# KenanGokdenizAcet/phase-based-motion-manipulation

Hardware: AMD Instinct MI355X
Metric: magnified frames/sec at 1920×1080, 5-level pyramid; achieved HBM GB/s vs peak (higher is better)
Workload: dtype f32

## Files before the change

### phase-based-motion-manipulation_amd/csrc/mm_fft.hpp

```cpp
#pragma once
#include <hip/hip_runtime.h>

namespace mm {

typedef float c2 __attribute__((ext_vector_type(2)));

__host__ __device__ __forceinline__ c2 mk(float x, float y) { c2 r = {x, y}; return r; }
__device__ __forceinline__ c2 add(c2 a, c2 b) { return a + b; }
__device__ __forceinline__ c2 sub(c2 a, c2 b) { return a - b; }
__device__ __forceinline__ c2 scale(c2 a, float s) { return a * s; }

template <int DIR>
__device__ __forceinline__ c2 add_i(c2 x, c2 y)
{
    c2 d;
    if constexpr (DIR > 0)
        asm("v_pk_add_f32 %0, %1, %2 op_sel:[0,1] op_sel_hi:[1,0] neg_lo:[0,1]" : "=v"(d) : "v"(x), "v"(y));
    else
        asm("v_pk_add_f32 %0, %1, %2 op_sel:[0,1] op_sel_hi:[1,0] neg_hi:[0,1]" : "=v"(d) : "v"(x), "v"(y));
    return d;
}
template <int DIR>
__device__ __forceinline__ c2 sub_i(c2 x, c2 y) { return add_i<-DIR>(x, y); }

// ... 45 lines not shown
    x0 = s0 + s1;
    x2 = s0 - s1;
    x1 = add_i<DIR>(d0, t);
    x3 = sub_i<DIR>(d0, t);
}

template <int DIR>
__device__ __forceinline__ void dft8(c2 *v)
{
    constexpr float h = 0.70710678118654752f;
    c2 a0 = v[0] + v[4], b0 = v[0] - v[4];
    c2 a1 = v[1] + v[5], b1 = v[1] - v[5];
    c2 a2 = v[2] + v[6], b2 = v[2] - v[6];
    c2 a3 = v[3] + v[7], b3 = v[3] - v[7];
    b1 = add_i<DIR>(b1, b1) * h;
    b3 = sub_i<DIR>(b3, b3) * (-h);
    dft4<DIR>(a0, a1, a2, a3);
    const c2 s0 = add_i<DIR>(b0, b2), d0 = sub_i<DIR>(b0, b2);
    const c2 s1 = b1 + b3, t = b1 - b3;
    v[0] = a0; v[2] = a1; v[4] = a2; v[6] = a3;
    v[1] = s0 + s1;
    v[5] = s0 - s1;
    v[3] = add_i<DIR>(d0, t);
    v[7] = sub_i<DIR>(d0, t);
}

template <int R, int DIR>
__device__ __forceinline__ void apply_twiddles(c2 *u, c2 w1)
{
    if constexpr (R >= 2) u[1] = mul_tw<DIR>(u[1], w1);
    if constexpr (R >= 4) {
        const c2 w2 = mul(w1, w1);
        const c2 w3 = mul(w2, w1);
        u[2] = mul_tw<DIR>(u[2], w2);
        u[3] = mul_tw<DIR>(u[3], w3);
        if constexpr (R >= 8) {
            const c2 w4 = mul(w2, w2);
            u[4] = mul_tw<DIR>(u[4], w4);
            u[5] = mul_tw<DIR>(u[5], mul(w1, w4));
            u[6] = mul_tw<DIR>(u[6], mul(w2, w4));
            u[7] = mul_tw<DIR>(u[7], mul(w3, w4));
            if constexpr (R >= 16) {
                const c2 w8 = mul(w4, w4);
                u[8] = mul_tw<DIR>(u[8], w8);
                u[9] = mul_tw<DIR>(u[9], mul(w1, w8));
                u[10] = mul_tw<DIR>(u[10], mul(w2, w8));
                u[11] = mul_tw<DIR>(u[11], mul(w3, w8));
                const c2 w12 = mul(w4, w8);
                u[12] = mul_tw<DIR>(u[12], w12);
                u[13] = mul_tw<DIR>(u[13], mul(w1, w12));
                u[14] = mul_tw<DIR>(u[14], mul(w2, w12));
                u[15] = mul_tw<DIR>(u[15], mul(w3, w12));
            }
        }
    }
}

constexpr int fft_passes_v(int log2n) { return log2n / 3 + (log2n % 3 ? 1 : 0); }
constexpr int kTwSlots = 20;
template <int LOG2N> constexpr int fft_passes() { return fft_passes_v(LOG2N); }
constexpr int pass_radix_v(int log2n, int p) { return (p < log2n / 3) ? 8 : (log2n % 3 == 2 ? 4 : 2); }
template <int LOG2N, int P> constexpr int pass_radix() { return pass_radix_v(LOG2N, P); }
constexpr int pass_ns_v(int log2n, int p) { return p == 0 ? 1 : pass_ns_v(log2n, p - 1) * pass_radix_v(log2n, p - 1); }

constexpr int tw_entries_v(int log2n) { return 1 << log2n; }

template <int LOG2N, int P = 1, int TWST = 1>
__device__ __forceinline__ void preload_twiddles(c2 (&wb)[kTwSlots], int t, const c2 *__restrict__ tw)
{
    if constexpr (P < fft_passes<LOG2N>()) {
        constexpr int N = 1 << LOG2N, T = N / 8, R = pass_radix<LOG2N, P>(), B = 8 / R;
        constexpr int NS = pass_ns_v(LOG2N, P), TWS = N / (NS * R);
#pragma unroll
        for (int q = 0; q < B; ++q) wb[P * 4 + q] = tw[((t + q * T) & (NS - 1)) * TWS * TWST];
        preload_twiddles<LOG2N, P + 1, TWST>(wb, t, tw);
    }
}

constexpr int xpad_s(int log2n, int ns) { return log2n < 9 || ns == 1 ? 3 : (ns == 8 ? 5 : 30); }
constexpr int xpad_a(int log2n, int ns) { return log2n < 9 || ns == 1 ? 1 : (ns == 8 ? 4 : 0); }
template <int LOG2N, int NS>
__host__ __device__ constexpr int xpad(int i) { return i + xpad_a(LOG2N, NS) * (i >> xpad_s(LOG2N, NS)); }

template <bool WSYNC>
__device__ __forceinline__ void xsync()
{
    if constexpr (WSYNC) __builtin_amdgcn_wave_barrier();
    else __syncthreads();
}

template <int LOG2N, int P, int DIR, bool WSYNC = false>
__device__ __forceinline__ void fft_pass(c2 (&v)[8], int t, c2 *lds, const c2 (&wb)[kTwSlots])
{
    constexpr int N = 1 << LOG2N, T = N / 8, R = pass_radix<LOG2N, P>(), B = 8 / R;
    constexpr int NS = pass_ns_v(LOG2N, P);
    constexpr bool LAST = P == fft_passes<LOG2N>() - 1;
#pragma unroll
    for (int q = 0; q < B; ++q) {
        const int b = t + q * T;
        c2 u[R];
#pragma unroll
        for (int m = 0; m < R; ++m) u[m] = v[q + m * B];
        if constexpr (NS > 1) apply_twiddles<R, DIR>(u, wb[P * 4 + q]);
        if constexpr (R == 8) dft8<DIR>(u);
        else if constexpr (R == 4) dft4<DIR>(u[0], u[1], u[2], u[3]);
        else dft2<DIR>(u[0], u[1]);
        if constexpr (LAST) {
#pragma unroll
            for (int m = 0; m < R; ++m) v[q + m * B] = u[m];
        } else {
            c2 *row = lds + xpad<LOG2N, NS>((b / NS) * NS * R + (b & (NS - 1)));
#pragma unroll
            for (int m = 0; m < R; ++m) row[xpad<LOG2N, NS>(m * NS)] = u[m];
        }
    }
    if constexpr (!LAST) {
        xsync<WSYNC>();
        if constexpr (T % 32 == 0) {
            const c2 *col = lds + xpad<LOG2N, NS>(t);
#pragma unroll
            for (int j = 0; j < 8; ++j) v[j] = lds_ld(col + xpad<LOG2N, NS>(j * T));
        } else {
#pragma unroll
            for (int j = 0; j < 8; ++j) v[j] = lds_ld(lds + xpad<LOG2N, NS>(t + j * T));
        }
        xsync<WSYNC>();
    }
}

template <int LOG2N, int DIR, int P, bool WSYNC = false>
__device__ __forceinline__ void fft_pass_loop(c2 (&v)[8], int t, c2 *lds, const c2 (&wb)[kTwSlots])
{
    if constexpr (P < fft_passes<LOG2N>()) {
        fft_pass<LOG2N, P, DIR, WSYNC>(v, t, lds, wb);
        fft_pass_loop<LOG2N, DIR, P + 1, WSYNC>(v, t, lds, wb);
    }
}

template <int LOG2N, int DIR>
__device__ __forceinline__ void fft_regs(c2 (&v)[8], int t, c2 *lds, const c2 *__restrict__ tw)
{
    c2 wb[kTwSlots];
    preload_twiddles<LOG2N>(wb, t, tw);
    fft_pass_loop<LOG2N, DIR, 0>(v, t, lds, wb);
}

constexpr bool tw_slot_used(int log2n, int i)
{
    return i / 4 >= 1 && i / 4 < fft_passes_v(log2n) && i % 4 < 8 / pass_radix_v(log2n, i / 4);
}

template <int LOG2N, int DIR>
__device__ __forceinline__ void fft_regs_w(c2 (&v)[8], int t, c2 *lds, const c2 (&wf)[kTwSlots])
{
    fft_pass_loop<LOG2N, DIR, 0>(v, t, lds, wf);
}

constexpr int fft_c_v(int log2n) { return log2n >= 9 && log2n <= 12 ? 1 << (log2n - 9) : 1; }
constexpr int fft_inner_v(int log2n) { return log2n >= 9 ? 9 : log2n; }
constexpr int fft_region_v(int log2n) { return (1 << fft_inner_v(log2n)) + (1 << fft_inner_v(log2n)) / 8; }

constexpr bool tw_slot_used_wl(int log2n, int i)
{
    return fft_c_v(log2n) == 1 ? tw_slot_used(log2n, i)
                               : (i == 4 || i == 8 || (i >= 12 && i < 12 + 8 / fft_c_v(log2n)));
}

template <int LOG2N>
__device__ __forceinline__ int fft_bin(int t, int j)
{
    constexpr int C = fft_c_v(LOG2N), T = (1 << LOG2N) / 8;
    if constexpr (C == 1) return t + j * T;
    else return (t >> 6) + C * ((t & 63) + 64 * j);
}

template <int LOG2N>
__host__ __device__ constexpr int zslot(int f)
{
    constexpr int C = fft_c_v(LOG2N), N = 1 << LOG2N;
    return C == 1 ? f : (f % C) * (N / C + 8) + f / C;
}
template <int LOG2N>
__host__ __device__ constexpr int zslot_h(int e)
{
    constexpr int C = fft_c_v(LOG2N), N = 1 << LOG2N;
    return C == 1 ? e : (e % C) * (N / (2 * C) + 8) + e / C;
}
template <int LOG2N> constexpr int zslot_h_size()
{
    return fft_c_v(LOG2N) == 1 ? (1 << LOG2N) / 2 + 1 : (1 << LOG2N) / 2 + 8 * fft_c_v(LOG2N);
}

template <int LOG2N>
__device__ __forceinline__ void preload_twiddles_wl(c2 (&wb)[kTwSlots], int t, const c2 *__restrict__ tw)
{
    constexpr int C = fft_c_v(LOG2N);
    if constexpr (C == 1) {
        preload_twiddles<LOG2N>(wb, t, tw);
    } else {
        preload_twiddles<9, 1, C>(wb, t & 63, tw);
#pragma unroll
        for (int h = 0; h < 8 / C; ++h) wb[12 + h] = tw[t + 64 * C * h];
    }
}

template <int C, int DIR>
__device__ __forceinline__ void dft_c(c2 *u)
{
    if constexpr (C == 8) dft8<DIR>(u);
    else if constexpr (C == 4) dft4<DIR>(u[0], u[1], u[2], u[3]);
    else dft2<DIR>(u[0], u[1]);
}

// ... 58 lines not shown
```

### phase-based-motion-manipulation_amd/csrc/mm_impl.hpp

```cpp
#pragma once
#if (defined(MM_K2_STAMPS) || defined(MM_K34_STAMPS)) && !defined(MM_ONLY_LOG2N)
#error "stamp builds are one-size builds: compile csrc/mm_api.hip alone with -DMM_ONLY_LOG2N=<log2 N>"
#endif
#include <hip/hip_runtime.h>

#include <algorithm>
#include <cmath>
#include <cstdio>
#include <cstdlib>
#include <cstring>
#include <new>
#include <vector>

#include "../../include/mm.h"
#include "mm_steer.hpp"

using namespace mm;

#define HIPCHK(x)                                                             \
    do {                                                                      \
        hipError_t e_ = (x);                                                  \
        if (e_ != hipSuccess) {                                               \
            if (getenv("MM_DEBUG"))                                           \
                fprintf(stderr, "mm355: %s failed: %s (%s:%d)\n", #x,         \
// ... 451 lines not shown
    }
    for (int i = 1; i < p.levels - 1; ++i) {
        volatile float num = (float)(i - 1), den = (float)(p.levels - 3);
        const float ratio = num / den;
        const float center = p.min_freq * powf(p.max_freq / p.min_freq, 1.0f - ratio);
        const float bwid = center * 0.5f;
        sp.lo[i] = center - bwid;
        sp.hi[i] = center + bwid;
        sp.inv_w[i] = 1.0f / (sp.hi[i] - sp.lo[i]);
    }
}

static bool bands_fit_table(const Spec &sp)
{
    for (int a = 1; a < sp.L - 1; ++a)
        for (int b = a + 1; b < sp.L - 1; ++b)
            for (int c = b + 1; c < sp.L - 1; ++c) {
                const float lo = fmaxf(sp.lo[a], fmaxf(sp.lo[b], sp.lo[c]));
                const float hi = fminf(sp.hi[a], fminf(sp.hi[b], sp.hi[c]));
                if (lo < hi) return false;
            }
    return true;
}

static bool bands_overlap(const Spec &sp)
{
    for (int a = 1; a < sp.L - 1; ++a)
        for (int b = a + 1; b < sp.L - 1; ++b) {
            const float lo = fmaxf(sp.lo[a], sp.lo[b]), hi = fminf(sp.hi[a], sp.hi[b]);
            if (hi - lo > 1e-5f * hi) return true;
        }
    return false;
}

static Blur5 build_blur()
{
    const double c0 = 0.2270270270, c1 = 0.3162162162, c2w = 0.0702702703;
    const double f1 = 0.5 * 1.3846153846, f2 = 0.5 * 3.2307692308 - 1.0;
    Blur5 b;
    b.w0 = (float)(c0 + 2.0 * c1 * (1.0 - f1));
    b.w1 = (float)(c1 * f1 + c2w * (1.0 - f2));
    b.w2 = (float)(c2w * f2);
    return b;
}

static int validate_params(const mm_params *p)
{
    if (!p) return MM_ERR_INVALID;
    if (p->levels < 1 || p->levels > kMaxLevels) return MM_ERR_UNSUPPORTED;
    if (p->mode == MM_MODE_STEERABLE) {
        if (p->orientations != 4 && p->orientations != 6 && p->orientations != 8)
            return MM_ERR_UNSUPPORTED;
        if (p->temporal_filter != MM_FILTER_DIFF && p->temporal_filter != MM_FILTER_IIR)
            return MM_ERR_INVALID;
        if (p->temporal_filter == MM_FILTER_IIR &&
            !(p->iir_low > 0.0f && p->iir_low < p->iir_high && p->iir_high <= 1.0f))
            return MM_ERR_INVALID;
    } else {
        if (p->orientations != 1) return MM_ERR_UNSUPPORTED;
        if (p->mode != MM_MODE_PYRAMID && p->mode != MM_MODE_STANDARD) return MM_ERR_UNSUPPORTED;
    }
    if (p->edge_mode != MM_EDGE_REPEAT && p->edge_mode != MM_EDGE_CLAMP) return MM_ERR_INVALID;
    if (!(p->min_freq > 0.0f) || !(p->max_freq > 0.0f)) return MM_ERR_INVALID;
    return MM_OK;
}

static constexpr int ktab_slots(int log2n)
{
    const int C = fft_c_v(log2n), te = (1 << log2n) / 2 + 1;
    return (te + C - 1) / C * C;
}

static int ilog2(int n)
{
    int l = 0;
    while ((1 << l) < n) ++l;
    return l;
}

template <int LOG2N> static size_t lds_fft_bytes()
{
    return sizeof(c2) * (size_t)groups_per_wg<LOG2N>() * lds_complex<(1 << LOG2N)>();
}
template <int LOG2N>
static int set_attrs(int W)
{
    (void)W;
    if constexpr (LOG2N == 12) {
        const int lds = (int)(sizeof(c2) * 2 * lds_complex<4096>());
        for (int f : {MM_RGBA8, MM_RGBA32F, MM_RGBA16F, MM_RGBA8_SRGB, MM_NV12, MM_P010, MM_Y8, MM_Y16, MM_YUY2})
            MM_FMT_SWITCH(f, HIPCHK(hipFuncSetAttribute(reinterpret_cast<const void *>(&k_rows_inv_compose<12, FMT_>),
                                                        hipFuncAttributeMaxDynamicSharedMemorySize, lds)))
        HIPCHK(hipFuncSetAttribute(reinterpret_cast<const void *>(&k_sb_cols<12>),
                                   hipFuncAttributeMaxDynamicSharedMemorySize, 81920));
    }
    if constexpr (LOG2N == 13) {
        auto set = [](const void *f, size_t b) {
            return b > 65536 ? hipFuncSetAttribute(f, hipFuncAttributeMaxDynamicSharedMemorySize, (int)b)
                             : hipSuccess;
        };
        const size_t x = sizeof(c2) * lds_complex<8192>();
        HIPCHK(set(reinterpret_cast<const void *>(&k_rows_inv<13>), sizeof(c2) * k3_groups<13>() * lds_complex<8192>()));
        HIPCHK(set(reinterpret_cast<const void *>(&k_dbg_cols<13>), 2 * sizeof(c2) * lds_complex<4096>()));
        (void)x;
#define MM_SET_K2(MODE)                                                                                  \
        HIPCHK(set(reinterpret_cast<const void *>(&k_cols<13, MODE>), k2_lds_bytes<13, MODE>()));        \
        HIPCHK(set(reinterpret_cast<const void *>(&k_cols_tail<13, MODE>), k2_lds_bytes<13, MODE>()))
        MM_SET_K2(MM_MODE_PYRAMID);
        MM_SET_K2(MM_MODE_STANDARD);
        MM_SET_K2(MM_K2_PYR_TAB);
#undef MM_SET_K2
    }
    if constexpr (LOG2N == 11) {
        const int lds = (int)(sizeof(c2) * 4 * lds_complex<2048>());
        for (int f : {MM_RGBA8, MM_RGBA32F, MM_RGBA16F, MM_RGBA8_SRGB, MM_NV12, MM_P010, MM_Y8, MM_Y16, MM_YUY2})
            MM_FMT_SWITCH(f, HIPCHK(hipFuncSetAttribute(reinterpret_cast<const void *>(&k_rows_inv_compose4<11, FMT_>),
                                                        hipFuncAttributeMaxDynamicSharedMemorySize, lds)))
    }
    return MM_OK;
}

template <int LOG2N>
static int launch_k1(mm_handle *h, const uint8_t *in, int nframes, const Frames &fr, hipStream_t s, c2 *G)
{
    const int fmt = fr.fmt;
    const int ppf = (h->H + 1) / 2;
    const int total = ppf * nframes;
    const bool lat = (total + k1_groups<LOG2N>() - 1) / k1_groups<LOG2N>() < 512;
    ProfScope ps(h, s, MM_K_ROWS_FWD, nframes);
#define MM_K1_LAUNCH(F, GEN, LAT)                                                                  \
    do {                                                                                           \
        constexpr int gpw = k1_gpw<LOG2N, LAT>();                                                  \
        const size_t lds = sizeof(c2) * (size_t)gpw * lds_complex<(1 << LOG2N)>();                \
        if (lds > 65536)                                                                           \
            HIPCHK(hipFuncSetAttribute(reinterpret_cast<const void *>(&k_rows_fwd<LOG2N, F, GEN, LAT>), \
                                       hipFuncAttributeMaxDynamicSharedMemorySize, (int)lds));     \
        hipLaunchKernelGGL((k_rows_fwd<LOG2N, F, GEN, LAT>), dim3((total + gpw - 1) / gpw),         \
                           dim3(gpw * fft_T<LOG2N>()), lds, s, in, ppf, total, g,                  \
                           h->d_col3, h->d_row3, h->d_col, h->d_row, h->d_tw, G, h->g_stride);     \
    } while (0)
    const bool gen = h->geo.ox || h->geo.oy;
    const Geo g = geo_of(h, fr);
    if (gen) {
        MM_FMT_SWITCH_FULLRES(fmt, MM_K1_LAUNCH(kK1Fmt<FMT_>, true, false))
    } else {
        MM_FMT_SWITCH_K1(fmt, if (lat) MM_K1_LAUNCH(kK1Fmt<FMT_>, false, true);
                              else MM_K1_LAUNCH(kK1Fmt<FMT_>, false, false))
    }
#undef MM_K1_LAUNCH
    HIPCHK(hipGetLastError());
    return MM_OK;
}

template <int LOG2N>
static int launch_k2(mm_handle *h, int nframes, const c2 *Gprev, const c2 *G, hipStream_t s)
{
    const int gpw = k2_groups<LOG2N>();
    const int cols = (1 << LOG2N) / 2;
    const int blocks = (cols + gpw - 1) / gpw;
    static_assert(ktab_slots(LOG2N) == k2_tab_slots<LOG2N>(), "d_ktab column stride");
    const int tab_mode = h->spec.mode == MM_MODE_STANDARD ? MM_MODE_STANDARD : h->k2_tab ? MM_K2_PYR_TAB : -1;
    if (tab_mode >= 0 && h->ktab_mode != tab_mode) {
        const int n = (cols + 1) * k2_tab_slots<LOG2N>();
        if (tab_mode == MM_MODE_STANDARD)
            hipLaunchKernelGGL((k_k2_table<LOG2N, MM_MODE_STANDARD>), dim3((n + 255) / 256), dim3(256), 0, s,
                               h->d_ktab, h->d_kmsum, h->spec);
        else
            hipLaunchKernelGGL((k_k2_table<LOG2N, MM_K2_PYR_TAB>), dim3((n + 255) / 256), dim3(256), 0, s,
                               h->d_ktab, h->d_kmsum, h->spec);
        HIPCHK(hipGetLastError());
        h->ktab_mode = tab_mode;
    }
    ProfScope ps(h, s, MM_K_COLS, nframes);
    int k = nframes >= 24 ? nframes * h->k2_tail_pct / 100 : 0;
    k = std::max(0, std::min(k, nframes - 2));
    const int k2t = nframes >= 24 && blocks >= 2 ? std::min(nframes * h->k2_tail2_pct / 100, nframes - 2) : 0;
    const int tb = k2t > 0 ? blocks / 2 : 0;
#define MM_K2_LAUNCH(MODE)                                                                           \
    do {                                                                                             \
                                         \
        const size_t lds = k2_lds_bytes<LOG2N, MODE>();                                              \
        hipLaunchKernelGGL((k_cols<LOG2N, MODE>), dim3(blocks + tb), dim3(k2_threads<LOG2N>()), lds, s, G, \
                           h->g_stride, Gprev, h->d_Q, h->q_stride, nframes, h->geo, h->spec, h->d_tw, h->d_ktab, \
                           h->d_kmsum, nframes - k, tb, k2t);                                        \
        if (k)                                                                                       \
            hipLaunchKernelGGL((k_cols_tail<LOG2N, MODE>), dim3(k), dim3(k2_threads<LOG2N>()), lds, s, G, \
                               h->g_stride, Gprev, h->d_Q, h->q_stride, nframes - k, h->geo, h->spec, h->d_tw, \
                               h->d_ktab, h->d_kmsum);                                               \
    } while (0)
    if (h->spec.mode == MM_MODE_STANDARD) MM_K2_LAUNCH(MM_MODE_STANDARD);
    else if (h->k2_tab2) MM_K2_LAUNCH(MM_K2_PYR_TAB2);
    else if (h->k2_tab) MM_K2_LAUNCH(MM_K2_PYR_TAB);
    else MM_K2_LAUNCH(MM_MODE_PYRAMID);
#undef MM_K2_LAUNCH
    HIPCHK(hipGetLastError());
    return MM_OK;
}

static int ensure_frames(mm_handle *h, void **buf, int *have, int frames, size_t per_frame, hipStream_t s)
{
    if (*buf && *have >= frames) return MM_OK;
    void *p = nullptr;
    if (h_alloc(h, &p, per_frame * (size_t)frames) != hipSuccess) return MM_ERR_OOM;
    h_retire(h, *buf, s, true);
    *buf = p;
    *have = frames;
    return MM_OK;
}
static int ensure_yh(mm_handle *h, hipStream_t s)
{
    return ensure_frames(h, reinterpret_cast<void **>(&h->d_Yh), &h->yh_frames, h->chunk,
                         sizeof(float) * h->yh_stride, s);
}

static int place_batch(mm_handle *h, int n, hipStream_t s, int *base)
{
    *base = 0;
    if (!h->g_valid) return MM_OK;
    if (h->gs + 1 + n <= h->chunk + 1) {
        *base = h->gs + 1;
        return MM_OK;
    }
    if (n > h->gs) {
        HIPCHK(hipMemcpyAsync(h->d_G + h->g_stride * h->chunk, h->d_G + h->g_stride * h->gs,
                              sizeof(c2) * h->g_stride, hipMemcpyDeviceToDevice, s));
        h->gs = h->chunk;
    }
    return MM_OK;
}

static int launch_k4(mm_handle *h, const uint8_t *in, uint8_t *out, int frame0, int nframes,
                     const Frames &fr, hipStream_t s);

static bool nv12_quads_aligned(const uint8_t *in, const uint8_t *out, const Frames &fr, int nframes)
{
    const uintptr_t a = reinterpret_cast<uintptr_t>(in) + fr.in.c_off, b = reinterpret_cast<uintptr_t>(out);
    uintptr_t m = a | fr.in.c_pitch | b | fr.out.pitch | (b + fr.out.c_off) | fr.out.c_pitch;
    if (nframes > 1) m |= fr.in.stride | fr.out.stride;
    return (m & 3u) == 0;
}
static bool mono_quads_aligned(const uint8_t *out, const Frames &fr, int nframes)
{
    uintptr_t m = reinterpret_cast<uintptr_t>(out) | fr.out.pitch;
    if (nframes > 1) m |= fr.out.stride;
    return (m & 3u) == 0;
}
static bool k34_fits(const mm_handle *h, const uint8_t *in, const uint8_t *out, const Frames &fr, int nframes)
{
    if (fmt_nv12(fr.fmt) && !nv12_quads_aligned(in, out, fr, nframes)) return false;
    if (fmt_mono(fr.fmt) && !mono_quads_aligned(out, fr, nframes)) return false;
    const Geo &g = h->geo;
    return g.N <= 4096 &&
           !g.ox && !g.oy && g.W % 8 == 0 && g.x0 >= 4 && g.x0 % 4 == 0 &&
           g.x0 + g.W + 4 <= g.N && g.N - g.H >= 4 && g.Hn == g.H + 4 && g.rb == g.y0 - 2 &&
           2 * (g.N / 8) >= g.W / 4;
}

#ifndef MM_K34_ROWS_4K
#define MM_K34_ROWS_4K 128
#endif
static int k34_strip_rows(const mm_handle *h, int nout)
{
    if (h->k34_rows >= 0) return h->k34_rows;
    const int cap = h->N >= 4096 ? MM_K34_ROWS_4K : 64;
    const int R = std::min(cap, (int)((long long)h->H * nout / 1024) / 4 * 4);
    return R >= 16 ? R : 0;
}

template <int LOG2N>
static int launch_k3(mm_handle *h, const uint8_t *in, uint8_t *out, int frame0, int nframes,
                     const Frames &fr, hipStream_t s)
{
    const int nout = nframes - frame0;
    if (nout <= 0) return MM_OK;
    const int fmt = fr.fmt;
    const int R = k34_strip_rows(h, nout);
    constexpr int k34o_per_cu = 4 * fft_T<LOG2N>() <= 1024 ? 1024 / (4 * fft_T<LOG2N>()) : 0;
    if constexpr (LOG2N <= 11) if (R == 0 && h->k34_rows < 0 && h->k34_oneshot && k34_fits(h, in, out, fr, nframes) &&
                                   ((LOG2N <= 10 && (h->H + 3) / 4 * nout <= k34o_per_cu * h->num_cu) ||
                                    h->k34_oneshot == 2)) {
        const int strips = (h->H + 3) / 4;
        const size_t lds = sizeof(c2) * 4 * lds_complex<(1 << LOG2N)>();
        const dim3 grid((unsigned)(strips * nout)), block(4 * fft_T<LOG2N>());
        ProfScope ps(h, s, MM_K_ROWS_INV_COMPOSE, nout);
        MM_FMT_SWITCH(fmt, hipLaunchKernelGGL((k_rows_inv_compose4<LOG2N, FMT_>), grid, block, lds, s, h->d_Q,
                                              h->q_stride, in, out, frame0, strips, geo_of(h, fr), h->blur,
                                              h->d_col3, h->d_row3, h->d_tw))
        HIPCHK(hipGetLastError());
        return MM_OK;
    }
    if (R >= 4 && k34_fits(h, in, out, fr, nframes)) {
        const int strips = (h->H + R - 1) / R, steps = R / 4 + 1;
        const size_t lds = sizeof(c2) * 2 * lds_complex<(1 << LOG2N)>();
        const dim3 grid((unsigned)(strips * nout)), block(2 * fft_T<LOG2N>());
        ProfScope ps(h, s, MM_K_ROWS_INV_COMPOSE, nout);
        MM_FMT_SWITCH(fmt, hipLaunchKernelGGL((k_rows_inv_compose<LOG2N, FMT_>), grid, block, lds, s, h->d_Q,
                                              h->q_stride, in, out, frame0, strips, steps, geo_of(h, fr),
                                              h->blur, h->d_col3, h->d_row3, h->d_tw))
        HIPCHK(hipGetLastError());
        return MM_OK;
    }
    const int ppf = h->geo.Hq / 2;
    const int total = ppf * nout;
    const int gpw = k3_groups<LOG2N>();
    int rc = ensure_yh(h, s);
    if (rc) return rc;
    {
        ProfScope ps(h, s, MM_K_ROWS_INV, nout);
        hipLaunchKernelGGL((k_rows_inv<LOG2N>), dim3((total + gpw - 1) / gpw),
                           dim3(k3_threads<LOG2N>()), sizeof(c2) * (size_t)gpw * lds_complex<(1 << LOG2N)>(),
                           s, h->d_Q,
                           h->q_stride, h->d_Yh, h->yh_stride, frame0, ppf, total, h->geo,
                           h->blur, h->d_tw);
        HIPCHK(hipGetLastError());
    }
    return launch_k4(h, in, out, frame0, nframes, fr, s);
}

template <int FMT> static constexpr auto k4_kernel()
{
    if constexpr (kMono<FMT>) return &k_compose_mono<FMT>;
    else return &k_compose<FMT>;
}
static int launch_k4(mm_handle *h, const uint8_t *in, uint8_t *out, int frame0, int nframes,
                     const Frames &fr, hipStream_t s)
{
    const int nout = nframes - frame0;
    if (nout <= 0) return MM_OK;
    const int fmt = fr.fmt;
    if (h->geo.ox || h->geo.oy) {
        const size_t tot = (size_t)nout * h->W * h->H;
        ProfScope ps(h, s, MM_K_COMPOSE, nout);
        const dim3 grid((unsigned)((tot + 255) / 256));
        MM_FMT_SWITCH_FULLRES(fmt, hipLaunchKernelGGL((k_compose_odd<FMT_>), grid, dim3(256), 0, s, h->d_Yh,
                                              h->yh_stride, in, out, frame0, nout, geo_of(h, fr), h->blur,
                                              h->d_col, h->d_row))
        HIPCHK(hipGetLastError());
        return MM_OK;
    }
    const int rt = (h->H + kTileRows - 1) / kTileRows, ct = (h->W + kTileCols - 1) / kTileCols;
    const dim3 grid(rt * ct * nout);
    ProfScope ps(h, s, MM_K_COMPOSE, nout);
    MM_FMT_SWITCH(fmt, hipLaunchKernelGGL((k4_kernel<FMT_>()), grid, dim3(kTileCols), 0, s, h->d_Yh,
                                          h->yh_stride, in, out, frame0, rt, ct, geo_of(h, fr), h->blur,
                                          h->d_col3, h->d_row3))
    HIPCHK(hipGetLastError());
    return MM_OK;
}

static int copy_frames(mm_handle *h, const uint8_t *in, uint8_t *out, int n, const Frames &fr, hipStream_t s)
{
    if (n <= 0) return MM_OK;
    if (fr.packed) {
        HIPCHK(hipMemcpyAsync(out, in, fr.fb * n, hipMemcpyDeviceToDevice, s));
        return MM_OK;
    }
    const unsigned rb = (unsigned)fmt_row_bytes(h->W, fr.fmt);
    const int rows = fmt_420(fr.fmt) ? h->H + h->H / 2 : h->H;
    const Geo g = geo_of(h, fr);
    for (int f0 = 0; f0 < n; f0 += 32768) {
        const dim3 grid((unsigned)rows, (unsigned)std::min(32768, n - f0));
        const uint8_t *src = in + fr.in.stride * f0;
        uint8_t *dst = out + fr.out.stride * f0;
        if (fmt_unit(fr.fmt) == 1) hipLaunchKernelGGL((k_copy_rows<uint8_t>), grid, dim3(256), 0, s, src, dst, g, rb, h->H);
        else if (fmt_unit(fr.fmt) == 2) hipLaunchKernelGGL((k_copy_rows<uint16_t>), grid, dim3(256), 0, s, src, dst, g, rb, h->H);
        else hipLaunchKernelGGL((k_copy_rows<uint32_t>), grid, dim3(256), 0, s, src, dst, g, rb, h->H);
        HIPCHK(hipGetLastError());
    }
    return MM_OK;
}

static int steer_bands(const mm_handle *h)
{
    const int nmid = h->spec.L >= 3 ? h->spec.L - 2 : 0;
    return nmid * (h->spec.O / 2);
}
static int steer_planes(const mm_handle *h) { return h->spec.filt == MM_FILTER_IIR ? 3 : 1; }
static size_t steer_plane_floats(const mm_handle *h)
{
    return (size_t)steer_bands(h) * h->geo.Hn * (h->geo.Wy + 4);
}
// ... 245 lines not shown
```

### phase-based-motion-manipulation_amd/csrc/mm_kernels.hpp

```cpp
#pragma once
#include "mm_fft.hpp"
#include "mm_srgb.hpp"
#include <stdint.h>
#include <type_traits>

namespace mm {

constexpr int kMaxLevels = 16;
constexpr float kPi = 3.14159265359f;

struct Tap4 {
    int idx[4];
    float w[4];
};

struct Geo {
    int W, H, N;
    int x0, y0;
    int ox, oy;
    int Hg;
    int Wy;
    int rb;
    int Hn;
    int Hq;
// ... 1839 lines not shown
                if (r % 2 == 0) {
                    cd0 = cd;
                } else {
                    const c2 v = cd0 + cd;
                    const float mine = X & 1 ? v.y : v.x, send = X & 1 ? v.x : v.y;
                    const float theirs = __builtin_bit_cast(float, __builtin_amdgcn_mov_dpp(
                        __builtin_bit_cast(int, send), 0xB1, 0xF, 0xF, true));
                    if constexpr (kP010<FMT>) {
                        const unsigned cc10 = p010_ccode(mine + theirs, X & 1 ? g.nv.cro : g.nv.cbo);
                        st_off<uint16_t>(outp, g.lo.c_off + (unsigned)(i >> 1) * g.lo.c_pitch + (unsigned)X * 2u,
                                         (uint16_t)(cc10 << 6));
                    } else {
                        const unsigned cc8 = nv12_ccode(mine + theirs, X & 1 ? g.nv.cro : g.nv.cbo);
                        st_off<uint8_t>(outp, g.lo.c_off + (unsigned)(i >> 1) * g.lo.c_pitch + (unsigned)X, (uint8_t)cc8);
                    }
                }
            } else if constexpr (k422<FMT>) {
                static_assert(TC % 2 == 0, "packed 4:2:2: tiles of whole macropixels");
                c2 cd;
                const unsigned yc = nv12_ycode(rr, gg, bb, g, cd);
                const float mine = X & 1 ? cd.y : cd.x, send = X & 1 ? cd.x : cd.y;
                const float theirs = __builtin_bit_cast(float, __builtin_amdgcn_mov_dpp(
                    __builtin_bit_cast(int, send), 0xB1, 0xF, 0xF, true));
                const unsigned cc = nv12_ccode(mine + theirs, X & 1 ? g.nv.cro : g.nv.cbo);
                const unsigned half = yc << (8u * g.lo.yb) | cc << (8u - 8u * g.lo.yb);
                const unsigned other = (unsigned)__builtin_amdgcn_mov_dpp((int)half, 0xB1, 0xF, 0xF, true);
                if (!(X & 1))
                    st_stream<uint32_t>(outp + (size_t)((unsigned)i * g.lo.pitch), (unsigned)X * 2u, half | other << 16);
            } else {
                Pix<FMT>::store(outp + (unsigned)i * g.lo.pitch, (unsigned)X, rr, gg, bb);
            }
        }
    }
}

template <int FMT>
__global__ __launch_bounds__(kTileCols)
void k_compose_mono(const float *__restrict__ Yh, size_t yh_stride, const uint8_t *__restrict__,
                    uint8_t *__restrict__ frames_out, int frame0, int row_tiles,
                    int col_tiles, Geo g, Blur5 bw, const float4 *__restrict__,
                    const float4 *__restrict__)
{
    static_assert(kMono<FMT>, "the 4:2:0 and RGBA formats compose with k_compose");
    constexpr int TR = kTileRows, TC = kTileCols;
    int b = blockIdx.x;
    const int ct = b % col_tiles;
    b /= col_tiles;
    const int rt = b % row_tiles;
    const int frame = frame0 + b / row_tiles;
    const int i0 = rt * TR, X = ct * TC + (int)threadIdx.x;
    if (X >= g.W) return;
    const float *Yf = Yh + (size_t)frame * yh_stride;
    float yv[TR + 4];
#pragma unroll
    for (int v = 0; v < TR + 4; ++v) {
        const int cy = wrap_near(g.y0 + i0 - 2 + v, g.N, g.edge);
        const int k = (cy - g.rb + 2 * g.N) & (g.N - 1);
        const float y = ld_off<float>(Yf, (unsigned)(min(k, g.Hn - 1) * g.Wy + X) * 4u);
        yv[v] = k < g.Hn ? y : 0.0f;
    }
    uint8_t *outp = frames_out + (size_t)frame * g.lo.stride;
#pragma unroll
    for (int r = 0; r < TR; ++r) {
        const int i = i0 + r;
        if (i < g.H) {
            const float yb = bw.w0 * yv[r + 2] + bw.w1 * (yv[r + 1] + yv[r + 3]) +
                             bw.w2 * (yv[r] + yv[r + 4]);
            mono_store<FMT>(outp + (size_t)((unsigned)i * g.lo.pitch), (unsigned)X, sat(yb), g);
        }
    }
}

#ifdef MM_K34_STAMPS
__device__ unsigned long long mm_k34_stamps[65536 * 8];
#define K34_STAMP(i)                                                     \
    do {                                                                 \
        const unsigned long long n_ = __builtin_amdgcn_s_memtime();      \
        st_acc[i] += n_ - st_prev;                                       \
        st_prev = n_;                                                    \
    } while (0)
#else
#define K34_STAMP(i) do { } while (0)
#endif
template <int LOG2N, int FMT>
__global__ __launch_bounds__(2 * fft_T<LOG2N>()) __attribute__((amdgpu_waves_per_eu(4)))
void k_rows_inv_compose(const c2 *__restrict__ Q, size_t q_stride,
                        const uint8_t *__restrict__ frames_in, uint8_t *__restrict__ frames_out,
                        int frame0, int strips, int steps, Geo g, Blur5 bw,
                        const float4 *__restrict__ colW3, const float4 *__restrict__ rowW3,
                        const c2 *__restrict__ tw)
{
    constexpr int N = 1 << LOG2N, T = fft_T<LOG2N>(), TK = q_tile<LOG2N>();
    using raw_t = typename ChromaSrc<FMT>::raw_t;
    constexpr unsigned bpp = LumaSrc<FMT>::bpp;
    extern __shared__ __attribute__((aligned(16))) c2 lds_all[];
    const int grp = T % 64 == 0 ? __builtin_amdgcn_readfirstlane(threadIdx.x / T) : threadIdx.x / T;
    const int t = threadIdx.x % T;
    c2 *lds = lds_all + grp * lds_complex<N>();
    const float *raw_all = reinterpret_cast<const float *>(lds_all);
    constexpr int GROUP_FLOATS = 2 * lds_complex<N>();
    const int b = xcd_remap(blockIdx.x, gridDim.x);
    const int frame = frame0 + b / strips;
    const int i0 = (b % strips) * 4 * (steps - 1);
    const c2 *Qf = Q + (size_t)frame * q_stride;
    const uint8_t *img = frames_in + (size_t)frame * g.li.stride;
    uint8_t *outp = frames_out + (size_t)frame * g.lo.stride;

    const int q = threadIdx.x;
    const bool vq = 4 * q < g.W;
    const int X = vq ? 4 * q : g.W - 4;
    const unsigned cl = (unsigned)wrap_near(X - 1, g.W, g.edge);
    const unsigned cr = (unsigned)wrap_near(X + 4, g.W, g.edge);
    auto chroma_row = [&](int i, c2 (&hc)[4]) {
        if constexpr (!kMono<FMT>) {
            const int row = wrap_near(min(i, g.H), g.H, g.edge);
            c2 a[6];
            if constexpr (k422<FMT>) {
                c422_quad_iq(img, g, row, (unsigned)X, cl, cr, a);
            } else if constexpr (k420<FMT>) {
                const unsigned pl = ld_off<raw_t>(img, c420_off<FMT>(g, row, cl));
                unsigned pm0, pm1;
                c420_quad_pairs<FMT>(img, g, row, (unsigned)X, pm0, pm1);
                const unsigned pr = ld_off<raw_t>(img, c420_off<FMT>(g, row, cr));
                a[0] = c420_iq2<FMT>(pl, g);
                a[1] = a[2] = c420_iq2<FMT>(pm0, g);
                a[3] = a[4] = c420_iq2<FMT>(pm1, g);
                a[5] = c420_iq2<FMT>(pr, g);
            } else {
                const unsigned base = (unsigned)row * (g.li.pitch / bpp);
                raw_t p[6];
                p[0] = ld_off<raw_t>(img, (base + cl) * bpp);
                if constexpr (bpp == 4) {
                    const uint4 m = ld_quad_a4(img, (base + (unsigned)X) * bpp);
                    p[1] = m.x; p[2] = m.y; p[3] = m.z; p[4] = m.w;
                } else {
#pragma unroll
                    for (int k = 0; k < 4; ++k) p[1 + k] = ld_off<raw_t>(img, (base + (unsigned)X + k) * bpp);
                }
                p[5] = ld_off<raw_t>(img, (base + cr) * bpp);
#pragma unroll
                for (int k = 0; k < 6; ++k) a[k] = chroma_iq2<FMT>(p[k]);
            }
#pragma unroll
            for (int k = 0; k < 4; ++k) {
                const float4 wc = colW3[X + k];
                hc[k] = wc.x * a[k] + wc.y * a[k + 1] + wc.z * a[k + 2];
            }
        }
    };

    float yw[8][4];
    [[maybe_unused]] c2 hc[6][4];
    chroma_row(i0 - 1, hc[4]);
    chroma_row(i0, hc[5]);
#ifdef MM_K34_STAMPS
    unsigned long long st_acc[8] = {0, 0, 0, 0, 0, 0, 0, 0};
    unsigned long long st_prev = __builtin_amdgcn_s_memtime();
    st_acc[7] = __builtin_amdgcn_s_memrealtime();
#endif
    float4 qv[8];
    auto load_q = [&](int s_) {
        const int ka_ = i0 + 4 * s_ + 2 * grp;
        const int kl = ka_ < g.Hn ? ka_ : 0;
        const float4 *Qp = reinterpret_cast<const float4 *>(Qf + (size_t)(kl / TK) * g.Qs * TK + (kl % TK));
        const unsigned up = (unsigned)t * (TK / 2), dn = (unsigned)(T - 1 - t) * (TK / 2);
#pragma unroll
        for (int j = 0; j < 8; ++j) {
            if (j < 4) qv[j] = (Qp + (size_t)(j * T) * (TK / 2))[up];
            else qv[j] = (Qp + (size_t)(N - j * T - (T - 1)) * (TK / 2))[dn];
        }
    };
    for (int s = 0; s < steps; ++s) {
        const int ka = i0 + 4 * s + 2 * grp;
        const bool valid = ka < g.Hn;
        load_q(s);
        c2 v[8];
#pragma unroll
        for (int j = 0; j < 8; ++j) {
            const int fq = t + j * T;
            const bool mirror = fq > N / 2;
            const int ff = mirror ? N - fq : fq;
            float4 qq = qv[j];
            if (ff == 0 || ff == N / 2) { qq.y = 0.0f; qq.w = 0.0f; }
            if (mirror) { qq.y = -qq.y; qq.w = -qq.w; }
            v[j] = valid ? mk(qq.x - qq.w, qq.y + qq.z) : mk(0.0f, 0.0f);
        }
        K34_STAMP(0);
        fft_regs<LOG2N, +1>(v, t, lds, tw);
        K34_STAMP(1);
        float *raw = reinterpret_cast<float *>(lds) + kZShift;
#pragma unroll
        for (int j = 0; j < 8; ++j) {
            raw[t + j * T] = fabsf(v[j].x);
            raw[N + t + j * T] = fabsf(v[j].y);
        }
        __syncthreads();
        K34_STAMP(2);
        const float4 *b4 = reinterpret_cast<const float4 *>(raw_all) + ((g.x0 + X) >> 2);
#pragma unroll
        for (int r = 0; r < 4; ++r) {
            const float4 *r4 = b4 + ((r >> 1) * GROUP_FLOATS + (r & 1) * N) / 4;
            const float4 P = r4[0], Z = r4[1];
            yw[4 + r][0] = bw.w0 * P.z + bw.w1 * (P.y + P.w) + bw.w2 * (P.x + Z.x);
            yw[4 + r][1] = bw.w0 * P.w + bw.w1 * (P.z + Z.x) + bw.w2 * (P.y + Z.y);
            yw[4 + r][2] = bw.w0 * Z.x + bw.w1 * (P.w + Z.y) + bw.w2 * (P.z + Z.z);
            yw[4 + r][3] = bw.w0 * Z.y + bw.w1 * (Z.x + Z.z) + bw.w2 * (P.w + Z.w);
        }
        __syncthreads();
        K34_STAMP(3);
        if (s > 0) {
            if constexpr (k420<FMT>) {
#pragma unroll
                for (int k = 0; k < 4; ++k) hc[2][k] = hc[1][k];
                chroma_row(i0 + 4 * s - 2, hc[3]);
#pragma unroll
                for (int k = 0; k < 4; ++k) hc[4][k] = hc[3][k];
                chroma_row(i0 + 4 * s, hc[5]);
            } else {
#pragma unroll
                for (int r = 0; r < 4; ++r) chroma_row(i0 + 4 * s - 3 + r, hc[2 + r]);
            }
            [[maybe_unused]] c2 cd0[4];
            for (int r = 0; r < 4; ++r) {
                K34_STAMP(4);
                const int i = i0 + 4 * s - 4 + r;
                if constexpr (kMono<FMT>) {
                    if (vq && i < g.H) {
                        float yl[4];
#pragma unroll
                        for (int k = 0; k < 4; ++k) {
                            const float yb = bw.w0 * yw[r + 2][k] + bw.w1 * (yw[r + 1][k] + yw[r + 3][k]) +
                                             bw.w2 * (yw[r][k] + yw[r + 4][k]);
                            yl[k] = sat(yb);
                        }
                        mono_store_quad<FMT>(outp + (size_t)((unsigned)i * g.lo.pitch), (unsigned)X, yl, g);
                    }
                } else if (vq && i < g.H) {
                    const float4 wr = rowW3[i];
                    float rr[4], gg[4], bb[4];
#pragma unroll
                    for (int k = 0; k < 4; ++k) {
                        const c2 cc = wr.x * hc[r][k] + wr.y * hc[r + 1][k] + wr.z * hc[r + 2][k];
                        const float yb = bw.w0 * yw[r + 2][k] + bw.w1 * (yw[r + 1][k] + yw[r + 3][k]) +
                                         bw.w2 * (yw[r][k] + yw[r + 4][k]);
                        yiq_rgb(yb, cc, rr[k], gg[k], bb[k]);
                    }
                    [[maybe_unused]] const unsigned o = (unsigned)i * (g.lo.pitch / bpp) + (unsigned)X;
                    if constexpr (k422<FMT>) {
                        c422_store_quad(outp, g, i, X, rr, gg, bb);
                    } else if constexpr (k420<FMT>) {
                        c420_store_quad<FMT>(outp, g, i, X, r & 1, rr, gg, bb, cd0);
                    } else if constexpr (bpp == 4) {
                        uint4 px;
                        px.x = Pix<FMT>::pack(rr[0], gg[0], bb[0]);
                        px.y = Pix<FMT>::pack(rr[1], gg[1], bb[1]);
                        px.z = Pix<FMT>::pack(rr[2], gg[2], bb[2]);
                        px.w = Pix<FMT>::pack(rr[3], gg[3], bb[3]);
                        st_stream_quad_a4(outp + (size_t)((unsigned)i * g.lo.pitch), (unsigned)X * 4u, px);
                    } else {
#pragma unroll
                        for (int k = 0; k < 4; ++k) Pix<FMT>::store(outp, o + k, rr[k], gg[k], bb[k]);
                    }
                }
            }
        }
        K34_STAMP(5);
#pragma unroll
        for (int r = 0; r < 4; ++r)
#pragma unroll
            for (int k = 0; k < 4; ++k) yw[r][k] = yw[4 + r][k];
        if constexpr (!kMono<FMT>) {
#pragma unroll
            for (int k = 0; k < 4; ++k) {
                hc[0][k] = hc[4][k];
                hc[1][k] = hc[5][k];
            }
        }
    }
#ifdef MM_K34_STAMPS
    st_acc[6] = (unsigned long long)steps;
    st_acc[7] = (__builtin_amdgcn_s_memrealtime() - st_acc[7]) << 32 | (st_acc[7] & 0xffffffffull);
    const int w = blockIdx.x * (blockDim.x / 64) + threadIdx.x / 64;
    if (threadIdx.x % 64 == 0 && w < 65536)
        for (int i = 0; i < 8; ++i) mm_k34_stamps[w * 8 + i] = st_acc[i];
#endif
}

template <int LOG2N, int FMT>
__global__ __launch_bounds__(4 * fft_T<LOG2N>())
void k_rows_inv_compose4(const c2 *__restrict__ Q, size_t q_stride,
                         const uint8_t *__restrict__ frames_in, uint8_t *__restrict__ frames_out,
                         int frame0, int strips, Geo g, Blur5 bw,
                         const float4 *__restrict__ colW3, const float4 *__restrict__ rowW3,
                         const c2 *__restrict__ tw)
{
    constexpr int N = 1 << LOG2N, T = fft_T<LOG2N>(), TK = q_tile<LOG2N>();
    using raw_t = typename ChromaSrc<FMT>::raw_t;
    constexpr unsigned bpp = LumaSrc<FMT>::bpp;
    extern __shared__ __attribute__((aligned(16))) c2 lds_all[];
    const int grp = T % 64 == 0 ? __builtin_amdgcn_readfirstlane(threadIdx.x / T) : threadIdx.x / T;
// ... 332 lines not shown
```

Before: 54330.

## Stage RGBA8 source rows into LDS via async global_load_lds during FFT

For RGBA8/sRGB inputs with 16-byte-aligned pitches at N<=4096, the inverse-compose kernel issues global_load_lds DMA for the four upcoming source rows right after the first FFT pass. Chroma reconstruction then reads those rows from LDS, so the global-load latency overlaps with the remaining FFT passes. The FFT syncs become explicit lgkmcnt waits plus s_barrier, so the pending vmcnt DMA is not drained early. In exchange the kernel uses more LDS per workgroup, which may lower occupancy, and it relies on hand-placed waitcnt ordering.

After: 55520 (median of 6 runs). +2.2%, better.

```diff
diff --git a/phase-based-motion-manipulation_amd/csrc/mm_fft.hpp b/phase-based-motion-manipulation_amd/csrc/mm_fft.hpp
--- a/phase-based-motion-manipulation_amd/csrc/mm_fft.hpp
+++ b/phase-based-motion-manipulation_amd/csrc/mm_fft.hpp
@@ -151,14 +151,19 @@
 template <int LOG2N, int NS>
 __host__ __device__ constexpr int xpad(int i) { return i + xpad_a(LOG2N, NS) * (i >> xpad_s(LOG2N, NS)); }
 
-template <bool WSYNC>
+constexpr int kSyncLds = 2;
+template <int WSYNC>
 __device__ __forceinline__ void xsync()
 {
-    if constexpr (WSYNC) __builtin_amdgcn_wave_barrier();
+    if constexpr (WSYNC == kSyncLds) {
+        asm volatile("s_waitcnt lgkmcnt(0)" ::: "memory");
+        __builtin_amdgcn_s_barrier();
+        asm volatile("" ::: "memory");
+    } else if constexpr (WSYNC) __builtin_amdgcn_wave_barrier();
     else __syncthreads();
 }
 
-template <int LOG2N, int P, int DIR, bool WSYNC = false>
+template <int LOG2N, int P, int DIR, int WSYNC = 0>
 __device__ __forceinline__ void fft_pass(c2 (&v)[8], int t, c2 *lds, const c2 (&wb)[kTwSlots])
 {
     constexpr int N = 1 << LOG2N, T = N / 8, R = pass_radix<LOG2N, P>(), B = 8 / R;
@@ -197,7 +202,7 @@
     }
 }
 
-template <int LOG2N, int DIR, int P, bool WSYNC = false>
+template <int LOG2N, int DIR, int P, int WSYNC = 0>
 __device__ __forceinline__ void fft_pass_loop(c2 (&v)[8], int t, c2 *lds, const c2 (&wb)[kTwSlots])
 {
     if constexpr (P < fft_passes<LOG2N>()) {
diff --git a/phase-based-motion-manipulation_amd/csrc/mm_impl.hpp b/phase-based-motion-manipulation_amd/csrc/mm_impl.hpp
--- a/phase-based-motion-manipulation_amd/csrc/mm_impl.hpp
+++ b/phase-based-motion-manipulation_amd/csrc/mm_impl.hpp
@@ -557,12 +557,23 @@
 {
     return sizeof(c2) * (size_t)groups_per_wg<LOG2N>() * lds_complex<(1 << LOG2N)>();
 }
+template <int LOG2N> static size_t k34_lds_bytes(bool srcdma)
+{
+    return sizeof(c2) * 2 * lds_complex<(1 << LOG2N)>() + (srcdma ? (size_t)k34_src_bytes<LOG2N>() : 0);
+}
 template <int LOG2N>
 static int set_attrs(int W)
 {
     (void)W;
+    if constexpr (LOG2N <= 12) if (k34_lds_bytes<LOG2N>(true) > 65536) {
+        const int lds = (int)k34_lds_bytes<LOG2N>(true);
+        HIPCHK(hipFuncSetAttribute(reinterpret_cast<const void *>(&k_rows_inv_compose<LOG2N, MM_RGBA8, true>),
+                                   hipFuncAttributeMaxDynamicSharedMemorySize, lds));
+        HIPCHK(hipFuncSetAttribute(reinterpret_cast<const void *>(&k_rows_inv_compose<LOG2N, MM_RGBA8_SRGB, true>),
+                                   hipFuncAttributeMaxDynamicSharedMemorySize, lds));
+    }
     if constexpr (LOG2N == 12) {
-        const int lds = (int)(sizeof(c2) * 2 * lds_complex<4096>());
+        const int lds = (int)k34_lds_bytes<12>(false);
         for (int f : {MM_RGBA8, MM_RGBA32F, MM_RGBA16F, MM_RGBA8_SRGB, MM_NV12, MM_P010, MM_Y8, MM_Y16, MM_YUY2})
             MM_FMT_SWITCH(f, HIPCHK(hipFuncSetAttribute(reinterpret_cast<const void *>(&k_rows_inv_compose<12, FMT_>),
                                                         hipFuncAttributeMaxDynamicSharedMemorySize, lds)))
@@ -720,6 +731,13 @@
     if (nframes > 1) m |= fr.out.stride;
     return (m & 3u) == 0;
 }
+static bool k34_src_dma(const uint8_t *in, const Frames &fr, int nframes)
+{
+    if (fr.fmt != MM_RGBA8 && fr.fmt != MM_RGBA8_SRGB) return false;
+    uintptr_t m = reinterpret_cast<uintptr_t>(in) | fr.in.pitch;
+    if (nframes > 1) m |= fr.in.stride;
+    return (m & 15u) == 0;
+}
 static bool k34_fits(const mm_handle *h, const uint8_t *in, const uint8_t *out, const Frames &fr, int nframes)
 {
     if (fmt_nv12(fr.fmt) && !nv12_quads_aligned(in, out, fr, nframes)) return false;
@@ -766,12 +784,20 @@
     }
     if (R >= 4 && k34_fits(h, in, out, fr, nframes)) {
         const int strips = (h->H + R - 1) / R, steps = R / 4 + 1;
-        const size_t lds = sizeof(c2) * 2 * lds_complex<(1 << LOG2N)>();
+        const bool dma = LOG2N <= 12 && k34_src_dma(in, fr, nframes);
+        const size_t lds = k34_lds_bytes<LOG2N>(dma);
         const dim3 grid((unsigned)(strips * nout)), block(2 * fft_T<LOG2N>());
         ProfScope ps(h, s, MM_K_ROWS_INV_COMPOSE, nout);
-        MM_FMT_SWITCH(fmt, hipLaunchKernelGGL((k_rows_inv_compose<LOG2N, FMT_>), grid, block, lds, s, h->d_Q,
-                                              h->q_stride, in, out, frame0, strips, steps, geo_of(h, fr),
-                                              h->blur, h->d_col3, h->d_row3, h->d_tw))
+#define MM_K34_LAUNCH(F, DMA)                                                                        \
+        hipLaunchKernelGGL((k_rows_inv_compose<LOG2N, F, DMA>), grid, block, lds, s, h->d_Q,          \
+                           h->q_stride, in, out, frame0, strips, steps, geo_of(h, fr), h->blur,      \
+                           h->d_col3, h->d_row3, h->d_tw)
+        if constexpr (LOG2N <= 12) if (dma) {
+            if (fmt == MM_RGBA8) MM_K34_LAUNCH(MM_RGBA8, true);
+            else MM_K34_LAUNCH(MM_RGBA8_SRGB, true);
+        }
+        if (!dma) MM_FMT_SWITCH(fmt, MM_K34_LAUNCH(FMT_, false))
+#undef MM_K34_LAUNCH
         HIPCHK(hipGetLastError());
         return MM_OK;
     }
diff --git a/phase-based-motion-manipulation_amd/csrc/mm_kernels.hpp b/phase-based-motion-manipulation_amd/csrc/mm_kernels.hpp
--- a/phase-based-motion-manipulation_amd/csrc/mm_kernels.hpp
+++ b/phase-based-motion-manipulation_amd/csrc/mm_kernels.hpp
@@ -1945,7 +1945,9 @@
 #else
 #define K34_STAMP(i) do { } while (0)
 #endif
-template <int LOG2N, int FMT>
+template <int FMT> constexpr bool k34_dma_fmt = FMT == MM_RGBA8 || FMT == MM_RGBA8_SRGB;
+template <int LOG2N> constexpr int k34_src_bytes() { return 4 * 4 * (1 << LOG2N); }
+template <int LOG2N, int FMT, bool SRCDMA = false>
 __global__ __launch_bounds__(2 * fft_T<LOG2N>()) __attribute__((amdgpu_waves_per_eu(4)))
 void k_rows_inv_compose(const c2 *__restrict__ Q, size_t q_stride,
                         const uint8_t *__restrict__ frames_in, uint8_t *__restrict__ frames_out,
@@ -1956,7 +1958,10 @@
     constexpr int N = 1 << LOG2N, T = fft_T<LOG2N>(), TK = q_tile<LOG2N>();
     using raw_t = typename ChromaSrc<FMT>::raw_t;
     constexpr unsigned bpp = LumaSrc<FMT>::bpp;
-    extern __shared__ __attribute__((aligned(16))) c2 lds_all[];
+    static_assert(!SRCDMA || k34_dma_fmt<FMT>, "staged source rows: 4-byte pixels");
+    extern __shared__ __attribute__((aligned(16))) c2 lds_raw[];
+    [[maybe_unused]] const uint8_t *srcl = reinterpret_cast<const uint8_t *>(lds_raw);
+    c2 *lds_all = lds_raw + (SRCDMA ? k34_src_bytes<LOG2N>() / (int)sizeof(c2) : 0);
     const int grp = T % 64 == 0 ? __builtin_amdgcn_readfirstlane(threadIdx.x / T) : threadIdx.x / T;
     const int t = threadIdx.x % T;
     c2 *lds = lds_all + grp * lds_complex<N>();
@@ -2011,6 +2016,35 @@
             }
         }
     };
+    [[maybe_unused]] auto stage_row = [&](int i, int r) {
+        if constexpr (SRCDMA) {
+            typedef __attribute__((address_space(1))) const void gptr_t;
+            typedef __attribute__((address_space(3))) void lptr_t;
+            const int row = i < g.H ? i : (g.edge ? g.H - 1 : 0);
+            const uint8_t *src = img + (size_t)((unsigned)row * g.li.pitch) + (unsigned)X * 4u;
+            const unsigned wbase = (unsigned)__builtin_amdgcn_readfirstlane((int)(threadIdx.x & ~63u)) * 16u;
+            const uint8_t *dst = srcl + r * (4 * N) + wbase;
+            __builtin_amdgcn_global_load_lds((gptr_t *)src, (lptr_t *)dst, 16, 0, 0);
+        }
+    };
+    [[maybe_unused]] auto chroma_row_staged = [&](int r, c2 (&hc)[4]) {
+        if constexpr (SRCDMA) {
+            const uint8_t *rowp = srcl + r * (4 * N);
+            unsigned p[6];
+            p[0] = *reinterpret_cast<const unsigned *>(rowp + cl * 4u);
+            const uint4 m = *reinterpret_cast<const uint4 *>(rowp + (unsigned)X * 4u);
+            p[1] = m.x; p[2] = m.y; p[3] = m.z; p[4] = m.w;
+            p[5] = *reinterpret_cast<const unsigned *>(rowp + cr * 4u);
+            c2 a[6];
+#pragma unroll
+            for (int k = 0; k < 6; ++k) a[k] = chroma_iq2<FMT>(p[k]);
+#pragma unroll
+            for (int k = 0; k < 4; ++k) {
+                const float4 wc = colW3[X + k];
+                hc[k] = wc.x * a[k] + wc.y * a[k + 1] + wc.z * a[k + 2];
+            }
+        }
+    };
 
     float yw[8][4];
     [[maybe_unused]] c2 hc[6][4];
@@ -2049,7 +2083,18 @@
             v[j] = valid ? mk(qq.x - qq.w, qq.y + qq.z) : mk(0.0f, 0.0f);
         }
         K34_STAMP(0);
-        fft_regs<LOG2N, +1>(v, t, lds, tw);
+        if constexpr (SRCDMA) {
+            c2 wb[kTwSlots];
+            preload_twiddles<LOG2N>(wb, t, tw);
+            fft_pass<LOG2N, 0, +1>(v, t, lds, wb);
+            if (s > 0) {
+#pragma unroll
+                for (int r = 0; r < 4; ++r) stage_row(i0 + 4 * s - 3 + r, r);
+            }
+            fft_pass_loop<LOG2N, +1, 1, kSyncLds>(v, t, lds, wb);
+        } else {
+            fft_regs<LOG2N, +1>(v, t, lds, tw);
+        }
         K34_STAMP(1);
         float *raw = reinterpret_cast<float *>(lds) + kZShift;
 #pragma unroll
@@ -2057,18 +2102,29 @@
             raw[t + j * T] = fabsf(v[j].x);
             raw[N + t + j * T] = fabsf(v[j].y);
         }
-        __syncthreads();
+        xsync<SRCDMA ? kSyncLds : 0>();
         K34_STAMP(2);
         const float4 *b4 = reinterpret_cast<const float4 *>(raw_all) + ((g.x0 + X) >> 2);
 #pragma unroll
         for (int r = 0; r < 4; ++r) {
             const float4 *r4 = b4 + ((r >> 1) * GROUP_FLOATS + (r & 1) * N) / 4;
-            const float4 P = r4[0], Z = r4[1];
+            float4 P, Z;
+            if constexpr (SRCDMA) {
+                typedef float f32x4 __attribute__((ext_vector_type(4)));
+                typedef __attribute__((address_space(3))) const volatile f32x4 lds_vf4;
+                const f32x4 p = *(lds_vf4 *)(r4), z = *(lds_vf4 *)(r4 + 1);
+                P = make_float4(p.x, p.y, p.z, p.w);
+                Z = make_float4(z.x, z.y, z.z, z.w);
+            } else {
+                P = r4[0];
+                Z = r4[1];
+            }
             yw[4 + r][0] = bw.w0 * P.z + bw.w1 * (P.y + P.w) + bw.w2 * (P.x + Z.x);
             yw[4 + r][1] = bw.w0 * P.w + bw.w1 * (P.z + Z.x) + bw.w2 * (P.y + Z.y);
             yw[4 + r][2] = bw.w0 * Z.x + bw.w1 * (P.w + Z.y) + bw.w2 * (P.z + Z.z);
             yw[4 + r][3] = bw.w0 * Z.y + bw.w1 * (Z.x + Z.z) + bw.w2 * (P.w + Z.w);
         }
+        if constexpr (SRCDMA) asm volatile("s_waitcnt vmcnt(0)" ::: "memory");
         __syncthreads();
         K34_STAMP(3);
         if (s > 0) {
@@ -2079,6 +2135,9 @@
 #pragma unroll
                 for (int k = 0; k < 4; ++k) hc[4][k] = hc[3][k];
                 chroma_row(i0 + 4 * s, hc[5]);
+            } else if constexpr (SRCDMA) {
+#pragma unroll
+                for (int r = 0; r < 4; ++r) chroma_row_staged(r, hc[2 + r]);
             } else {
 #pragma unroll
                 for (int r = 0; r < 4; ++r) chroma_row(i0 + 4 * s - 3 + r, hc[2 + r]);
```
